# yanx27/PointASNL

Hardware: AMD Instinct MI355X
Metric: point-clouds/sec fwd (Bx1024 pts, ModelNet40 cls) (higher is better)
Workload: dtype f32; 1 GPU; configs[1]: ModelNet40 pointasnl_cls, 1024 pts, batch=64/GPU, seeded random weights; global_batch=64, parallelism=batch-shard x1, RCCL all-gather of logits, pipeline=prefetch, hip_graph=True, prefix_forked_at=start, prefix_levels=2, settle_replays=40, hip_hw_queues=4

## Files before the change

### pointasnl_amd/csrc/grouping.hip

```cpp
#include <math.h>
#include <stdlib.h>
#include <algorithm>
#include "common.hpp"

namespace pasnl {

constexpr int SEARCH_TILE = 2048;
constexpr int SEARCH_WAVES = 4;

__device__ __forceinline__ void stage_tile(const float* __restrict__ cloud, int n, int base, int cnt, float* sx, float* sy,
                                           float* sz) {
  const float* src = cloud + (size_t)base * 3;
  for (int f = threadIdx.x; f < cnt * 3; f += SEARCH_WAVES * 64) {
    float v = src[f];
    int p = f / 3, c = f - p * 3;
    (c == 0 ? sx : (c == 1 ? sy : sz))[p] = v;
  }
}

template <int QW>
__global__ __launch_bounds__(SEARCH_WAVES * 64) void ball_query_kernel(int n, int m, float thr2, int nsample,
                                                                      const float* __restrict__ xyz1,
                                                                      const float* __restrict__ xyz2,
                                                                      int* __restrict__ idx, int* __restrict__ pts_cnt) {
  extern __shared__ __attribute__((aligned(16))) char smem[];
  float* sx = reinterpret_cast<float*>(smem);
  float* sy = sx + SEARCH_TILE;
  float* sz = sy + SEARCH_TILE;
  int* hits = reinterpret_cast<int*>(sz + SEARCH_TILE);

  const int lane = threadIdx.x & 63, wave = threadIdx.x >> 6;
  const int bi = blockIdx.y;
  const float* cloud = xyz1 + (size_t)bi * n * 3;
  const int q0 = (blockIdx.x * SEARCH_WAVES + wave) * QW;

  float qx[QW], qy[QW], qz[QW];
  int cnt[QW], first[QW];
#pragma unroll
  for (int q = 0; q < QW; ++q) {
    int j = q0 + q;
    bool ok = j < m;
    const float* p = xyz2 + ((size_t)bi * m + (ok ? j : 0)) * 3;
    qx[q] = p[0]; qy[q] = p[1]; qz[q] = p[2];
    cnt[q] = ok ? 0 : nsample;
    first[q] = 0;
  }

  for (int base = 0; base < n; base += SEARCH_TILE) {
    int tcnt = min(SEARCH_TILE, n - base);
    __syncthreads();
    stage_tile(cloud, n, base, tcnt, sx, sy, sz);
    __syncthreads();
#pragma unroll
    for (int q = 0; q < QW; ++q) {
      int c = cnt[q];
      if (c >= nsample) continue;
      int* hq = hits + (size_t)(wave * QW + q) * nsample;
      for (int it = 0; it < tcnt; it += 64) {
        int p = it + lane;
        bool in = p < tcnt;
        float d2 = dist2(qx[q], qy[q], qz[q], in ? sx[p] : 0.f, in ? sy[p] : 0.f, in ? sz[p] : 0.f);
        bool hit = in && (d2 < thr2);
        unsigned long long mask = __ballot(hit);
        if (mask) {
          if (c == 0) first[q] = base + it + (int)__builtin_ctzll(mask);
          int rank = __builtin_amdgcn_mbcnt_hi((unsigned)(mask >> 32), __builtin_amdgcn_mbcnt_lo((unsigned)mask, 0u));
          int slot = c + rank;
          if (hit && slot < nsample) hq[slot] = base + it + lane;
          c += (int)__builtin_popcountll(mask);
          if (c >= nsample) { c = nsample; break; }
        }
      }
      cnt[q] = c;
    }
  }
#pragma unroll
  for (int q = 0; q < QW; ++q) {
    int j = q0 + q;
    if (j >= m) continue;
    const int* hq = hits + (size_t)(wave * QW + q) * nsample;
    int* o = idx + ((size_t)bi * m + j) * nsample;
    int c = cnt[q], pad = c > 0 ? first[q] : 0;
    for (int s = lane; s < nsample; s += 64) o[s] = s < c ? hq[s] : pad;
    if (lane == 0) pts_cnt[(size_t)bi * m + j] = c;
  }
}

int ball_grid_launch(int b, int n, int m, float radius, float thr2, int nsample, const float* xyz1, const float* xyz2, int* idx,
                     int* pts_cnt, hipStream_t stream);

template <int SLOTS>
struct KnnList {
  float d[SLOTS];
  int i[SLOTS];
};

template <int SLOTS>
__device__ __forceinline__ void knn_insert(KnnList<SLOTS>& L, float cd, int ck, int lane) {
  int pos = 0;
#pragma unroll
  for (int s = 0; s < SLOTS; ++s) pos += (int)__builtin_popcountll(__ballot(L.d[s] <= cd));
  float carry_d = 0.f;
  int carry_i = 0;
#pragma unroll
  for (int s = 0; s < SLOTS; ++s) {
    float top_d = readlane_f(L.d[s], 63);
    int top_i = __builtin_amdgcn_readlane(L.i[s], 63);
    float sd = wave_shr1_f(L.d[s]);
    int si = wave_shr1_i(L.i[s]);
    if (lane == 0) { sd = carry_d; si = carry_i; }
    int r = s * 64 + lane;
    if (r > pos) { L.d[s] = sd; L.i[s] = si; }
    if (r == pos) { L.d[s] = cd; L.i[s] = ck; }
    carry_d = top_d;
    carry_i = top_i;
  }
}

template <int SLOTS, int QW, typename IdxT>
__global__ __launch_bounds__(SEARCH_WAVES * 64) void knn_kernel(int n, int m, int k, const float* __restrict__ support,
                                                               const float* __restrict__ queries, IdxT* __restrict__ idx,
                                                               float* __restrict__ dist_out, const KnnTieFlags flags) {
  __shared__ float sx[SEARCH_TILE], sy[SEARCH_TILE], sz[SEARCH_TILE];
  const int lane = threadIdx.x & 63, wave = threadIdx.x >> 6;
  const int bi = blockIdx.y;
  const float* cloud = support + (size_t)bi * n * 3;
  const int q0 = (blockIdx.x * SEARCH_WAVES + wave) * QW;

  float qx[QW], qy[QW], qz[QW], tau[QW];
  float tie_tau[QW];
  const bool flagging = flags.nflag != nullptr;
  KnnList<SLOTS> L[QW];
  const int ks = (k - 1) >> 6, kl = (k - 1) & 63;
#pragma unroll
  for (int q = 0; q < QW; ++q) {
    int j = min(q0 + q, m - 1);
    const float* p = queries + ((size_t)bi * m + j) * 3;
    qx[q] = p[0]; qy[q] = p[1]; qz[q] = p[2];
    tau[q] = INFINITY;
    tie_tau[q] = -1.f;
#pragma unroll
    for (int s = 0; s < SLOTS; ++s) { L[q].d[s] = INFINITY; L[q].i[s] = 0; }
  }

  for (int base = 0; base < n; base += SEARCH_TILE) {
    int tcnt = min(SEARCH_TILE, n - base);
    __syncthreads();
    stage_tile(cloud, n, base, tcnt, sx, sy, sz);
    __syncthreads();
    for (int it = 0; it < tcnt; it += 64) {
      int p = it + lane;
      bool in = p < tcnt;
      float x = in ? sx[p] : 0.f, y = in ? sy[p] : 0.f, z = in ? sz[p] : 0.f;
      float dq[QW];
      dist2_multi<QW>(qx, qy, qz, x, y, z, dq);
#pragma unroll
      for (int q = 0; q < QW; ++q) {
        float d = dq[q];
        unsigned long long mask = __ballot(in && d < tau[q]);
        if (flagging && __ballot(in && d == tau[q]) != 0ull) tie_tau[q] = tau[q];
        while (mask) {
          int src = (int)__builtin_ctzll(mask);
          mask &= mask - 1;
          float cd = readlane_f(d, src);
          if (cd < tau[q]) {
            knn_insert<SLOTS>(L[q], cd, base + it + src, lane);
            float t = INFINITY;
#pragma unroll
            for (int s = 0; s < SLOTS; ++s)
              if (s == ks) t = readlane_f(L[q].d[s], kl);
            if (t == tau[q]) tie_tau[q] = t;
            tau[q] = t;
          } else if (cd == tau[q]) {
            tie_tau[q] = cd;
          }
        }
      }
    }
  }
#pragma unroll
  for (int q = 0; q < QW; ++q) {
    int j = q0 + q;
    if (j >= m) continue;
    size_t o = ((size_t)bi * m + j) * k;
    bool tie = flagging && tie_tau[q] == tau[q];
#pragma unroll
    for (int s = 0; s < SLOTS; ++s) {
      int r = s * 64 + lane;
      if (r < k) {
        idx[o + r] = (IdxT)L[q].i[s];
        if (dist_out) dist_out[o + r] = L[q].d[s];
      }
      if (flagging) {
        float prev = wave_shr1_f(L[q].d[s]);
        if (lane == 0) prev = s > 0 ? readlane_f(L[q].d[s > 0 ? s - 1 : 0], 63) : -1.f;
        tie = tie || __ballot(r >= 1 && r < k && L[q].d[s] == prev) != 0ull;
      }
    }
    if (tie) knn_flag_query(flags, bi, m, j, lane);
  }
}

constexpr int KNN2_CAP = 128;

template <int R, int QW, typename IdxT>
__global__ __launch_bounds__(SEARCH_WAVES * 64) void knn2_kernel(int n, int m, int k, const float* __restrict__ support,
                                                                const float* __restrict__ queries, IdxT* __restrict__ idx,
                                                                float* __restrict__ dist_out, const KnnTieFlags flags) {
  __shared__ float sx[SEARCH_TILE], sy[SEARCH_TILE], sz[SEARCH_TILE];
  __shared__ unsigned long long cand[SEARCH_WAVES * QW][KNN2_CAP];
  const int lane = threadIdx.x & 63, wave = threadIdx.x >> 6;
  const int bi = blockIdx.y;
  const float* cloud = support + (size_t)bi * n * 3;
  const int q0 = (blockIdx.x * SEARCH_WAVES + wave) * QW;
  constexpr uint32_t INF_BITS = 0x7f800000u;

  float qx[QW], qy[QW], qz[QW];
  uint32_t m1[QW], m2[QW];
#pragma unroll
  for (int q = 0; q < QW; ++q) {
    int j = min(q0 + q, m - 1);
    const float* p = queries + ((size_t)bi * m + j) * 3;
    qx[q] = p[0]; qy[q] = p[1]; qz[q] = p[2];
    m1[q] = INF_BITS; m2[q] = INF_BITS;
  }
  for (int base = 0; base < n; base += SEARCH_TILE) {
    int tcnt = min(SEARCH_TILE, n - base);
    __syncthreads();
    stage_tile(cloud, n, base, tcnt, sx, sy, sz);
    __syncthreads();
    for (int it = 0; it < tcnt; it += 64) {
      int p = it + lane;
      bool in = p < tcnt;
      const float x = sx[p], y = sy[p], z = sz[p];
      float dq[QW];
      dist2_multi<QW>(qx, qy, qz, x, y, z, dq);
#pragma unroll
      for (int q = 0; q < QW; ++q) {
        uint32_t di = in ? __float_as_uint(dq[q]) : INF_BITS;
        if (R == 2) m2[q] = min(m2[q], max(m1[q], di));
        m1[q] = min(m1[q], di);
      }
    }
  }
  uint32_t U[QW];
#pragma unroll
  for (int q = 0; q < QW; ++q) {
    uint32_t mv[R];
    mv[0] = m1[q];
    if (R == 2) mv[1] = m2[q];
    wave_bitonic_sort<R, uint32_t>(mv, lane);
    uint32_t u = 0;
#pragma unroll
    for (int r = 0; r < R; ++r)
      if (r == ((k - 1) >> 6)) u = (uint32_t)__builtin_amdgcn_readlane((int)mv[r], (k - 1) & 63);
    U[q] = u;
  }
  int cnt[QW];
#pragma unroll
  for (int q = 0; q < QW; ++q) cnt[q] = 0;
  for (int base = 0; base < n; base += SEARCH_TILE) {
    int tcnt = min(SEARCH_TILE, n - base);
    if (n > SEARCH_TILE) {
      __syncthreads();
      stage_tile(cloud, n, base, tcnt, sx, sy, sz);
      __syncthreads();
    }
    for (int it = 0; it < tcnt; it += 64) {
      int p = it + lane;
      bool in = p < tcnt;
      const float x = sx[p], y = sy[p], z = sz[p];
      float dq[QW];
      dist2_multi<QW>(qx, qy, qz, x, y, z, dq);
#pragma unroll
      for (int q = 0; q < QW; ++q) {
        uint32_t di = __float_as_uint(dq[q]);
        bool c = in && di <= U[q];
        unsigned long long mask = __ballot(c);
        if (mask) {
          int rank = __builtin_amdgcn_mbcnt_hi((unsigned)(mask >> 32), __builtin_amdgcn_mbcnt_lo((unsigned)mask, 0u));
          int slot = cnt[q] + rank;
          if (c && slot < KNN2_CAP) cand[wave * QW + q][slot] = ((unsigned long long)di << 32) | (uint32_t)(base + p);
          cnt[q] += (int)__builtin_popcountll(mask);
        }
      }
    }
  }
  bool overflow = false;
#pragma unroll
  for (int q = 0; q < QW; ++q) {
    const int j = q0 + q;
    const int c = cnt[q];
    if (c > KNN2_CAP) { overflow = overflow || (j < m); continue; }
    if (j >= m) continue;
    const unsigned long long* cb = cand[wave * QW + q];
    const size_t o = ((size_t)bi * m + j) * k;
    if (c <= 64) {
      unsigned long long key[1];
      key[0] = lane < c ? cb[lane] : ~0ull;
      wave_bitonic_sort<1, unsigned long long>(key, lane);
      if (lane < k) {
        idx[o + lane] = (IdxT)(uint32_t)key[0];
        if (dist_out) dist_out[o + lane] = __uint_as_float((uint32_t)(key[0] >> 32));
      }
      if (flags.nflag && knn_sorted_has_tie(key[0], ~0ull, k, lane)) knn_flag_query(flags, bi, m, j, lane);
    } else {
      unsigned long long key[2];
      key[0] = cb[lane];
      key[1] = 64 + lane < c ? cb[64 + lane] : ~0ull;
      wave_bitonic_sort<2, unsigned long long>(key, lane);
      if (lane < k) {
        idx[o + lane] = (IdxT)(uint32_t)key[0];
        if (dist_out) dist_out[o + lane] = __uint_as_float((uint32_t)(key[0] >> 32));
      }
      if (flags.nflag && knn_sorted_has_tie(key[0], key[1], k, lane)) knn_flag_query(flags, bi, m, j, lane);
    }
  }
  if (!__syncthreads_or(overflow ? 1 : 0)) return;
  float tau[QW], tie_tau[QW];
  KnnList<1> L[QW];
  bool todo[QW];
#pragma unroll
  for (int q = 0; q < QW; ++q) {
    todo[q] = cnt[q] > KNN2_CAP && (q0 + q) < m;
    tau[q] = INFINITY;
    tie_tau[q] = -1.f;
    L[q].d[0] = INFINITY;
    L[q].i[0] = 0;
  }
  for (int base = 0; base < n; base += SEARCH_TILE) {
    int tcnt = min(SEARCH_TILE, n - base);
    __syncthreads();
    stage_tile(cloud, n, base, tcnt, sx, sy, sz);
    __syncthreads();
    for (int it = 0; it < tcnt; it += 64) {
      int p = it + lane;
      bool in = p < tcnt;
      float x = in ? sx[p] : 0.f, y = in ? sy[p] : 0.f, z = in ? sz[p] : 0.f;
#pragma unroll
      for (int q = 0; q < QW; ++q) {
        if (!todo[q]) continue;
        float d = dist2(qx[q], qy[q], qz[q], x, y, z);
        unsigned long long mask = __ballot(in && d < tau[q]);
        if (__ballot(in && d == tau[q]) != 0ull) tie_tau[q] = tau[q];
        while (mask) {
          int src = (int)__builtin_ctzll(mask);
          mask &= mask - 1;
          float cd = readlane_f(d, src);
          if (cd < tau[q]) {
            knn_insert<1>(L[q], cd, base + it + src, lane);
            const float t = readlane_f(L[q].d[0], k - 1);
            if (t == tau[q]) tie_tau[q] = t;
            tau[q] = t;
          } else if (cd == tau[q]) {
            tie_tau[q] = cd;
          }
        }
      }
    }
  }
#pragma unroll
  for (int q = 0; q < QW; ++q) {
    if (!todo[q]) continue;
    size_t o = ((size_t)bi * m + q0 + q) * k;
    if (lane < k) {
      idx[o + lane] = (IdxT)L[q].i[0];
      if (dist_out) dist_out[o + lane] = L[q].d[0];
    }
    if (flags.nflag) {
      const float prev = wave_shr1_f(L[q].d[0]);
      if (tie_tau[q] == tau[q] || __ballot(lane >= 1 && lane < k && L[q].d[0] == prev) != 0ull) knn_flag_query(flags, bi, m, q0 + q, lane);
    }
  }
}

template <int VEC>
__global__ __launch_bounds__(256) void group_point_kernel(int n, int c, long rows_per_batch, long total_chunks,
                                                         const float* __restrict__ points, const int* __restrict__ idx,
                                                         float* __restrict__ out) {
  const int cpr = c / VEC;
  for (long g = (long)blockIdx.x * 256 + threadIdx.x; g < total_chunks; g += (long)gridDim.x * 256) {
    long row = g / cpr;
    int ch = (int)(g - row * cpr);
    long bi = row / rows_per_batch;
    int a = idx[row];
    const float* src = points + ((size_t)bi * n + a) * c + (size_t)ch * VEC;
    float* dst = out + (size_t)row * c + (size_t)ch * VEC;
    if constexpr (VEC == 4) {
      *reinterpret_cast<float4*>(dst) = *reinterpret_cast<const float4*>(src);
    } else {
      *dst = *src;
    }
  }
}

__global__ __launch_bounds__(256) void group_point_grad_kernel(int n, int c, long rows_per_batch, long total,
                                                              const float* __restrict__ grad_out,
                                                              const int* __restrict__ idx, float* __restrict__ grad_points) {
  for (long e = (long)blockIdx.x * 256 + threadIdx.x; e < total; e += (long)gridDim.x * 256) {
    long row = e / c;
    int l = (int)(e - row * c);
    long bi = row / rows_per_batch;
    int a = idx[row];
    atomicAdd(&grad_points[((size_t)bi * n + a) * c + l], grad_out[e]);
  }
}

template <int T>
__global__ __launch_bounds__(T) void sa_group_kernel(int n, int c, int m, int k, const float* __restrict__ xyz,
                                                    const float* __restrict__ feature, const int* __restrict__ idx,
                                                    const float* __restrict__ new_xyz, float* __restrict__ new_point,
                                                    float* __restrict__ skip_max) {
  extern __shared__ __attribute__((aligned(16))) char smem[];
  int* sidx = reinterpret_cast<int*>(smem);
  float* part = reinterpret_cast<float*>(sidx + k);
  const int W = 6 + c;
  const int R = T / W;
  const long g = blockIdx.x;
  const long bi = g / m;
  const int t = threadIdx.x;
  for (int s = t; s < k; s += T) sidx[s] = idx[g * k + s];
  __syncthreads();
  const float* cx = xyz + (size_t)bi * n * 3;
  const float* cf = feature + (size_t)bi * n * c;
  float* out = new_point + (size_t)g * k * W;
  if (W > T) {
    for (int col = t; col < W; col += T) {
      const float centre = col < 3 ? new_xyz[g * 3 + col] : 0.f;
      float mx = -INFINITY;
      for (int s = 0; s < k; ++s) {
        const int i = sidx[s];
        float v;
        if (col < 3) v = cx[(size_t)i * 3 + col] - centre;
        else if (col < 6) v = cx[(size_t)i * 3 + (col - 3)];
        else v = cf[(size_t)i * c + (col - 6)];
        out[(size_t)s * W + col] = v;
        mx = fmaxf(mx, v);
      }
      skip_max[g * W + col] = mx;
    }
    return;
  }
  const int col = t % W, r0 = t / W;
  const bool active = r0 < R;
  float centre = 0.f;
  if (active && col < 3) centre = new_xyz[g * 3 + col];
  float mx = -INFINITY;
  if (active) {
    for (int s = r0; s < k; s += R) {
      const int i = sidx[s];
      float v;
      if (col < 3) v = cx[(size_t)i * 3 + col] - centre;
      else if (col < 6) v = cx[(size_t)i * 3 + (col - 3)];
      else v = cf[(size_t)i * c + (col - 6)];
      out[(size_t)s * W + col] = v;
      mx = fmaxf(mx, v);
    }
    part[r0 * W + col] = mx;
  }
  __syncthreads();
  if (t < W) {
    float v = part[t];
    for (int r = 1; r < R; ++r) v = fmaxf(v, part[r * W + t]);
    skip_max[g * W + t] = v;
  }
}

constexpr int GL_THREADS = 1024;

__global__ __launch_bounds__(GL_THREADS) void grad_lists_kernel(int n, long entries, const int* __restrict__ idx,
                                                               int* __restrict__ start, int* __restrict__ list) {
  extern __shared__ __attribute__((aligned(16))) char smem[];
  int* cnt = reinterpret_cast<int*>(smem);
  __shared__ int wsum[GL_THREADS / 64];
  const int tid = threadIdx.x, lane = tid & 63, wave = tid >> 6;
  const long bi = blockIdx.x;
  const int* ix = idx + bi * entries;
  for (int t = tid; t < n; t += GL_THREADS) cnt[t] = 0;
  __syncthreads();
  for (long e = tid; e < entries; e += GL_THREADS) {
    const int t = ix[e];
    if (t >= 0 && t < n) atomicAdd(&cnt[t], 1);
  }
  __syncthreads();
  const int per = (n + GL_THREADS - 1) / GL_THREADS;
  int sum = 0;
  for (int j = 0; j < per; ++j) {
    const int t = tid * per + j;
    if (t < n) sum += cnt[t];
  }
  int incl = sum;
#pragma unroll
  for (int off = 1; off < 64; off <<= 1) {
    int o = __shfl_up(incl, off);
    if (lane >= off) incl += o;
  }
  if (lane == 63) wsum[wave] = incl;
  __syncthreads();
  int base = incl - sum;
  for (int w = 0; w < wave; ++w) base += wsum[w];
  int* st = start + bi * (n + 1);
  for (int j = 0; j < per; ++j) {
    const int t = tid * per + j;
    if (t < n) {
      const int c = cnt[t];
      cnt[t] = base;
      st[t] = base;
      base += c;
    }
  }
  if (tid == GL_THREADS - 1) st[n] = base;
  __syncthreads();
  int* ls = list + bi * entries;
  for (long e = tid; e < entries; e += GL_THREADS) {
    const int t = ix[e];
    if (t >= 0 && t < n) ls[atomicAdd(&cnt[t], 1)] = (int)e;
  }
}

__global__ __launch_bounds__(256) void grad_segsum_kernel(int n, int c, long entries, int rep, const float* __restrict__ src,
                                                         const float* __restrict__ weight, const int* __restrict__ start,
                                                         const int* __restrict__ list, float* __restrict__ dst, long rows) {
  const int lane = threadIdx.x & 63;
  const long r = (long)blockIdx.x * 4 + (threadIdx.x >> 6);
  if (r >= rows) return;
  const long bi = r / n;
  const int t = (int)(r - bi * n);
  const int lo = start[bi * (n + 1) + t], hi = start[bi * (n + 1) + t + 1];
  const int* ls = list + bi * entries;
  float* out = dst + r * c;
  constexpr int CH = 8;
  for (int c0 = 0; c0 < c; c0 += CH * 64) {
    float acc[CH];
#pragma unroll
    for (int q = 0; q < CH; ++q) acc[q] = 0.f;
    uint32_t prev = 0;
    bool first = true;
    for (int done = lo; done < hi;) {
      uint32_t key[2];
      key[0] = 0xffffffffu;
      for (int base = lo; base < hi; base += 64) {
        uint32_t cand = 0xffffffffu;
        if (base + lane < hi) {
          const uint32_t e = (uint32_t)ls[base + lane];
          if (first || e > prev) cand = e;
        }
        key[1] = cand;
        wave_bitonic_sort<2, uint32_t>(key, lane);
      }
      const int take = min(64, hi - done);
      for (int j = 0; j < take; ++j) {
        const uint32_t e = (uint32_t)__builtin_amdgcn_readlane((int)key[0], j);
        const long ge = bi * entries + e;
        const float* row = src + (ge / rep) * c + c0 + lane;
        const float w = weight ? weight[ge] : 1.f;
#pragma unroll
        for (int q = 0; q < CH; ++q) {
          if (c0 + q * 64 + lane < c) {
            const float v = row[q * 64];
            acc[q] = acc[q] + (weight ? v * w : v);
          }
        }
      }
      prev = (uint32_t)__builtin_amdgcn_readlane((int)key[0], take - 1);
      first = false;
      done += take;
    }
#pragma unroll
    for (int q = 0; q < CH; ++q)
      if (c0 + q * 64 + lane < c) out[c0 + q * 64 + lane] = acc[q];
  }
}

__global__ __launch_bounds__(256) void take_neighbor0_kernel(int n, int c, int m, int k, long total, const float* __restrict__ xyz,
                                                            const float* __restrict__ feature, const int* __restrict__ idx,
                                                            float* __restrict__ new_xyz, float* __restrict__ new_feature) {
  const int w = 3 + c;
  for (long e = (long)blockIdx.x * 256 + threadIdx.x; e < total; e += (long)gridDim.x * 256) {
    const long row = e / w;
    const int col = (int)(e - row * w);
    const long bi = row / m;
    const int i = idx[row * k];
    const float v = col < 3 ? xyz[((size_t)bi * n + i) * 3 + col] : feature[((size_t)bi * n + i) * c + (col - 3)];
    new_feature[e] = v;
    if (col < 3) new_xyz[row * 3 + col] = v;
  }
}

__global__ __launch_bounds__(256) void max_pool_rows_kernel(int n, int c, const float* __restrict__ x, float* __restrict__ out,
                                                            long out_stride) {
  __shared__ float part[4][64];
  const int lane = threadIdx.x & 63, wave = threadIdx.x >> 6;
  const int col = blockIdx.x * 64 + lane;
  const bool ok = col < c;
  const float* p = x + (size_t)blockIdx.y * n * c + (ok ? col : 0);
  float m0 = -INFINITY, m1 = -INFINITY, m2 = -INFINITY, m3 = -INFINITY;
  int s = wave;
  for (; s + 12 < n; s += 16) {
    float a = p[(size_t)s * c], b = p[(size_t)(s + 4) * c], d = p[(size_t)(s + 8) * c], e = p[(size_t)(s + 12) * c];
    m0 = fmaxf(m0, a); m1 = fmaxf(m1, b); m2 = fmaxf(m2, d); m3 = fmaxf(m3, e);
  }
  for (; s < n; s += 4) m0 = fmaxf(m0, p[(size_t)s * c]);
  part[wave][lane] = fmaxf(fmaxf(m0, m1), fmaxf(m2, m3));
  __syncthreads();
  if (wave == 0 && ok)
    out[(size_t)blockIdx.y * out_stride + col] = fmaxf(fmaxf(part[0][lane], part[1][lane]), fmaxf(part[2][lane], part[3][lane]));
}

__global__ __launch_bounds__(256) void select_top_k_kernel(int n, int k, long rows, const float* __restrict__ dist,
                                                          int* __restrict__ outi, float* __restrict__ out) {
  const int lane = threadIdx.x & 63;
  long row = (long)blockIdx.x * 4 + (threadIdx.x >> 6);
  if (row >= rows) return;
  const float* src = dist + (size_t)row * n;
  float* pd = out + (size_t)row * n;
  int* pi = outi + (size_t)row * n;
  for (int s = lane; s < n; s += 64) { pd[s] = src[s]; pi[s] = s; }
  asm volatile("s_waitcnt vmcnt(0)" ::: "memory");
  for (int s = 0; s < k && s < n; ++s) {
    float bv = INFINITY;
    int bp = 0x7fffffff;
    for (int t = s + lane; t < n; t += 64) {
      float v = __hip_atomic_load(&pd[t], __ATOMIC_RELAXED, __HIP_MEMORY_SCOPE_AGENT);
      if (v < bv) { bv = v; bp = t; }
    }
#pragma unroll
    for (int off = 32; off >= 1; off >>= 1) {
      float ov = __shfl_xor(bv, off);
      int op = __shfl_xor(bp, off);
      if (ov < bv || (ov == bv && op < bp)) { bv = ov; bp = op; }
    }
    int mn = (bp == 0x7fffffff) ? s : bp;
    if (mn != s && lane == 0) {
      float vs = __hip_atomic_load(&pd[s], __ATOMIC_RELAXED, __HIP_MEMORY_SCOPE_AGENT);
      int is = __hip_atomic_load(&pi[s], __ATOMIC_RELAXED, __HIP_MEMORY_SCOPE_AGENT);
      int im = __hip_atomic_load(&pi[mn], __ATOMIC_RELAXED, __HIP_MEMORY_SCOPE_AGENT);
      __hip_atomic_store(&pd[mn], vs, __ATOMIC_RELAXED, __HIP_MEMORY_SCOPE_AGENT);
      __hip_atomic_store(&pd[s], bv, __ATOMIC_RELAXED, __HIP_MEMORY_SCOPE_AGENT);
      __hip_atomic_store(&pi[mn], is, __ATOMIC_RELAXED, __HIP_MEMORY_SCOPE_AGENT);
      __hip_atomic_store(&pi[s], im, __ATOMIC_RELAXED, __HIP_MEMORY_SCOPE_AGENT);
    }
    asm volatile("s_waitcnt vmcnt(0)" ::: "memory");
  }
}

}

using namespace pasnl;

static int grid_for(long total) {
  long g = (total + 255) / 256;
  return (int)(g < 1 ? 1 : (g > 8192 ? 8192 : g));
}

static float ball_threshold(float r) {
  float t = r * r;
  if (!(t < INFINITY)) return INFINITY;
  while (sqrtf(t) >= r && t > 0.f) t = nextafterf(t, -INFINITY);
  while (sqrtf(t) < r) t = nextafterf(t, INFINITY);
  return t;
}

extern "C" int pasnl_query_ball_point(int b, int n, int m, float radius, int nsample, const float* xyz1, const float* xyz2,
                                      int* idx, int* pts_cnt, pasnl_stream_t stream) {
  PASNL_REQUIRE(radius > 0.f, PASNL_EINVAL);
  PASNL_REQUIRE(nsample > 0, PASNL_EINVAL);
  PASNL_REQUIRE(b >= 0 && n > 0 && m >= 0, PASNL_EINVAL);
  if (b == 0 || m == 0) return PASNL_OK;
  PASNL_REQUIRE(xyz1 && xyz2 && idx && pts_cnt, PASNL_ENULL);
  PASNL_REQUIRE(b <= 65535, PASNL_EUNSUPPORTED);
  constexpr int QW = 4;
  float thr2 = (radius > 1e-20f) ? ball_threshold(radius) : 0.f;
  const int rc = ball_grid_launch(b, n, m, radius, thr2, nsample, xyz1, xyz2, idx, pts_cnt, pasnl_hip_stream(stream));
  if (rc != PASNL_EUNSUPPORTED) return rc;
  size_t lds = (size_t)SEARCH_TILE * 12 + (size_t)SEARCH_WAVES * QW * nsample * sizeof(int);
  PASNL_REQUIRE(lds <= LDS_MAX_BYTES, PASNL_EUNSUPPORTED);
  int qpb = SEARCH_WAVES * QW;
  if (launch(ball_query_kernel<QW>, dim3((m + qpb - 1) / qpb, b), dim3(SEARCH_WAVES * 64), lds, pasnl_hip_stream(stream), n, m, thr2,
             nsample, xyz1, xyz2, idx, pts_cnt) != PASNL_OK)
    return PASNL_ELAUNCH;
  return pasnl_launch_status();
}

template <int SLOTS, int QW>
static int knn_launch(int b, int n, int m, int k, const float* support, const float* queries, void* idx, int idx_is_i64,
                      float* dist2, pasnl::KnnTieFlags flags, hipStream_t st) {
  int qpb = SEARCH_WAVES * QW;
  dim3 grid((m + qpb - 1) / qpb, b), block(SEARCH_WAVES * 64);
  with_index_type(idx_is_i64, [&](auto tag) {
    using T = decltype(tag);
    hipLaunchKernelGGL((knn_kernel<SLOTS, QW, T>), grid, block, 0, st, n, m, k, support, queries, static_cast<T*>(idx), dist2, flags);
  });
  return pasnl_launch_status();
}

extern "C" int pasnl_knn_batch(int b, int n, int m, int k, const float* support, const float* queries, void* idx,
                               int idx_is_i64, float* dist2, pasnl_stream_t stream) {
  return pasnl::knn_brute_launch(b, n, m, k, support, queries, idx, idx_is_i64, dist2, pasnl::KnnTieFlags{nullptr, nullptr},
                                 pasnl_hip_stream(stream));
}

int pasnl::knn_brute_launch(int b, int n, int m, int k, const float* support, const float* queries, void* idx, int idx_is_i64,
                            float* dist2, pasnl::KnnTieFlags flags, hipStream_t st) {
  PASNL_REQUIRE(b >= 0 && n > 0 && m >= 0 && k > 0, PASNL_EINVAL);
  PASNL_REQUIRE(k <= n, PASNL_EINVAL);
  PASNL_REQUIRE(k <= PASNL_KNN_MAX_K, PASNL_EUNSUPPORTED);
  if (b == 0 || m == 0) return PASNL_OK;
  PASNL_REQUIRE(support && queries && idx, PASNL_ENULL);
  PASNL_REQUIRE(b <= 65535, PASNL_EUNSUPPORTED);
  if (k <= 64 && !(k <= 16 && n > 2048)) {
    const long nq = (long)b * m;
    constexpr long min_waves = 8192;
    const int qw = nq >= 4L * min_waves ? 4 : (nq >= 2L * min_waves ? 2 : 1);
    dim3 grid((m + SEARCH_WAVES * qw - 1) / (SEARCH_WAVES * qw), b), block(SEARCH_WAVES * 64);
    with_index_type(idx_is_i64, [&](auto tag) {
      using T = decltype(tag);
      auto kern = k <= 32 ? (qw == 4 ? knn2_kernel<1, 4, T> : qw == 2 ? knn2_kernel<1, 2, T> : knn2_kernel<1, 1, T>)
                          : (qw == 4 ? knn2_kernel<2, 4, T> : qw == 2 ? knn2_kernel<2, 2, T> : knn2_kernel<2, 1, T>);
      hipLaunchKernelGGL(kern, grid, block, 0, st, n, m, k, support, queries, static_cast<T*>(idx), dist2, flags);
    });
    return pasnl_launch_status();
  }
  if (k <= 64) return knn_launch<1, 4>(b, n, m, k, support, queries, idx, idx_is_i64, dist2, flags, st);
  if (k <= 128) return knn_launch<2, 2>(b, n, m, k, support, queries, idx, idx_is_i64, dist2, flags, st);
  return knn_launch<4, 1>(b, n, m, k, support, queries, idx, idx_is_i64, dist2, flags, st);
}

extern "C" int pasnl_group_point(int b, int n, int c, int m, int nsample, const float* points, const int* idx, float* out,
                                 pasnl_stream_t stream) {
  PASNL_REQUIRE(b >= 0 && n > 0 && c > 0 && m >= 0 && nsample >= 0, PASNL_EINVAL);
  long rows_per_batch = (long)m * nsample;
  long rows = (long)b * rows_per_batch;
  if (rows == 0) return PASNL_OK;
  PASNL_REQUIRE(points && idx && out, PASNL_ENULL);
  hipStream_t st = pasnl_hip_stream(stream);
  bool vec4 = (c % 4 == 0) && ((reinterpret_cast<uintptr_t>(points) | reinterpret_cast<uintptr_t>(out)) % 16 == 0);
  if (vec4) {
    long chunks = rows * (c / 4);
    hipLaunchKernelGGL(group_point_kernel<4>, dim3(grid_for(chunks)), dim3(256), 0, st, n, c, rows_per_batch, chunks, points,
                       idx, out);
  } else {
    long chunks = rows * c;
    hipLaunchKernelGGL(group_point_kernel<1>, dim3(grid_for(chunks)), dim3(256), 0, st, n, c, rows_per_batch, chunks, points,
                       idx, out);
  }
  return pasnl_launch_status();
}

extern "C" int pasnl_sa_group(int b, int n, int c, int m, int k, const float* xyz, const float* feature, const int* idx,
                              const float* new_xyz, float* new_point, float* skip_max, pasnl_stream_t stream) {
  PASNL_REQUIRE(b >= 0 && n > 0 && c > 0 && m >= 0 && k > 0, PASNL_EINVAL);
  const int W = 6 + c;
  long groups = (long)b * m;
  if (groups == 0) return PASNL_OK;
  PASNL_REQUIRE(groups < (1L << 31), PASNL_EUNSUPPORTED);
  PASNL_REQUIRE(xyz && feature && idx && new_xyz && new_point && skip_max, PASNL_ENULL);
  hipStream_t st = pasnl_hip_stream(stream);
  if (W <= 256) {
    size_t lds = (size_t)k * 4 + (size_t)(256 / W) * W * 4;
    if (launch(sa_group_kernel<256>, dim3((unsigned)groups), dim3(256), lds, st, n, c, m, k, xyz, feature, idx, new_xyz, new_point,
               skip_max) != PASNL_OK)
      return PASNL_ELAUNCH;
  } else {
    size_t lds = (size_t)k * 4 + (size_t)(W <= 512 ? (512 / W) * W : 0) * 4;
    if (launch(sa_group_kernel<512>, dim3((unsigned)groups), dim3(512), lds, st, n, c, m, k, xyz, feature, idx, new_xyz, new_point,
               skip_max) != PASNL_OK)
      return PASNL_ELAUNCH;
  }
  return pasnl_launch_status();
}

extern "C" int pasnl_group_point_grad(int b, int n, int c, int m, int nsample, const float* grad_out, const int* idx,
                                      float* grad_points, pasnl_stream_t stream) {
  PASNL_REQUIRE(b >= 0 && n > 0 && c > 0 && m >= 0 && nsample >= 0, PASNL_EINVAL);
  if (b == 0) return PASNL_OK;
  PASNL_REQUIRE(grad_points, PASNL_ENULL);
  hipStream_t st = pasnl_hip_stream(stream);
  if (hipMemsetAsync(grad_points, 0, (size_t)b * n * c * sizeof(float), st) != hipSuccess) return PASNL_ELAUNCH;
  long rows_per_batch = (long)m * nsample;
  long total = (long)b * rows_per_batch * c;
  if (total == 0) return PASNL_OK;
  PASNL_REQUIRE(grad_out && idx, PASNL_ENULL);
  hipLaunchKernelGGL(group_point_grad_kernel, dim3(grid_for(total)), dim3(256), 0, st, n, c, rows_per_batch, total, grad_out,
                     idx, grad_points);
  return pasnl_launch_status();
}

static size_t grad_ws_bytes(int b, int n, long entries) {
  return ((size_t)b * (n + 1) + (size_t)b * entries) * sizeof(int);
}

extern "C" size_t pasnl_grad_workspace_bytes(int b, int n, long entries) {
  if (b <= 0 || n <= 0 || entries < 0) return 0;
  return grad_ws_bytes(b, n, entries);
}

static int grad_det(int b, int n, int c, long entries, int rep, const float* src, const float* weight, const int* idx,
                    float* dst, void* ws, size_t ws_bytes, hipStream_t st) {
  PASNL_REQUIRE(b >= 0 && n > 0 && c > 0 && entries >= 0, PASNL_EINVAL);
  if (b == 0) return PASNL_OK;
  PASNL_REQUIRE(dst, PASNL_ENULL);
  PASNL_REQUIRE(entries == 0 || (src && idx), PASNL_ENULL);
  PASNL_REQUIRE(ws && ws_bytes >= grad_ws_bytes(b, n, entries), PASNL_EWORKSPACE);
  PASNL_REQUIRE((size_t)n * sizeof(int) <= 150 * 1024 && entries < (1L << 31), PASNL_EUNSUPPORTED);
  int* start = static_cast<int*>(ws);
  int* list = start + (size_t)b * (n + 1);
  size_t lds = (size_t)n * sizeof(int);
  if (launch(grad_lists_kernel, dim3(b), dim3(GL_THREADS), lds, st, n, entries, idx, start, list) != PASNL_OK) return PASNL_ELAUNCH;
  long rows = (long)b * n;
  hipLaunchKernelGGL(grad_segsum_kernel, dim3((unsigned)((rows + 3) / 4)), dim3(256), 0, st, n, c, entries, rep, src, weight, start,
                     list, dst, rows);
  return pasnl_launch_status();
}

extern "C" int pasnl_gather_point_grad_det(int b, int n, int m, const float* out_g, const int* idx, float* inp_g, void* ws,
                                           size_t ws_bytes, pasnl_stream_t stream) {
  PASNL_REQUIRE(m >= 0, PASNL_EINVAL);
  return grad_det(b, n, 3, m, 1, out_g, nullptr, idx, inp_g, ws, ws_bytes, pasnl_hip_stream(stream));
}

extern "C" int pasnl_group_point_grad_det(int b, int n, int c, int m, int nsample, const float* grad_out, const int* idx,
                                          float* grad_points, void* ws, size_t ws_bytes, pasnl_stream_t stream) {
  PASNL_REQUIRE(m >= 0 && nsample >= 0, PASNL_EINVAL);
  return grad_det(b, n, c, (long)m * nsample, 1, grad_out, nullptr, idx, grad_points, ws, ws_bytes, pasnl_hip_stream(stream));
}

extern "C" int pasnl_three_interpolate_grad_det(int b, int n, int c, int m, const float* grad_out, const int* idx,
                                                const float* weight, float* grad_points, void* ws, size_t ws_bytes,
                                                pasnl_stream_t stream) {
  PASNL_REQUIRE(n >= 0, PASNL_EINVAL);
  PASNL_REQUIRE(n == 0 || weight, PASNL_ENULL);
  return grad_det(b, m, c, 3L * n, 3, grad_out, weight, idx, grad_points, ws, ws_bytes, pasnl_hip_stream(stream));
}

extern "C" int pasnl_take_neighbor0(int b, int n, int c, int m, int k, const float* xyz, const float* feature, const int* idx,
                                    float* new_xyz, float* new_feature, pasnl_stream_t stream) {
  PASNL_REQUIRE(b >= 0 && n > 0 && c > 0 && m >= 0 && k > 0, PASNL_EINVAL);
  long total = (long)b * m * (3 + c);
  if (total == 0) return PASNL_OK;
  PASNL_REQUIRE(xyz && feature && idx && new_xyz && new_feature, PASNL_ENULL);
  hipLaunchKernelGGL(take_neighbor0_kernel, dim3(grid_for(total)), dim3(256), 0, pasnl_hip_stream(stream), n, c, m, k, total, xyz,
                     feature, idx, new_xyz, new_feature);
  return pasnl_launch_status();
}

extern "C" int pasnl_max_pool_rows_strided(int b, int n, int c, const float* x, float* out, long out_stride,
                                           pasnl_stream_t stream) {
  PASNL_REQUIRE(b >= 0 && n > 0 && c > 0 && out_stride >= c, PASNL_EINVAL);
  if (b == 0) return PASNL_OK;
  PASNL_REQUIRE(x && out, PASNL_ENULL);
  PASNL_REQUIRE(b <= 65535, PASNL_EUNSUPPORTED);
  hipLaunchKernelGGL(max_pool_rows_kernel, dim3((c + 63) / 64, b), dim3(256), 0, pasnl_hip_stream(stream), n, c, x, out,
                     out_stride);
  return pasnl_launch_status();
}

extern "C" int pasnl_max_pool_rows(int b, int n, int c, const float* x, float* out, pasnl_stream_t stream) {
  return pasnl_max_pool_rows_strided(b, n, c, x, out, c, stream);
}

extern "C" int pasnl_select_top_k(int b, int n, int m, int k, const float* dist, int* outi, float* out,
                                  pasnl_stream_t stream) {
  PASNL_REQUIRE(k > 0, PASNL_EINVAL);
  PASNL_REQUIRE(b >= 0 && n > 0 && m >= 0, PASNL_EINVAL);
  long rows = (long)b * m;
  if (rows == 0) return PASNL_OK;
  PASNL_REQUIRE(dist && outi && out, PASNL_ENULL);
  hipLaunchKernelGGL(select_top_k_kernel, dim3((unsigned)((rows + 3) / 4)), dim3(256), 0, pasnl_hip_stream(stream), n, k, rows,
                     dist, outi, out);
  return pasnl_launch_status();
}
```

Measured before the change: 58590 point-clouds/s.

## Keep kNN distances in registers for small clouds and compact candidates branch-free

For support clouds of up to 1024 points, the brute-force kNN kernel now loads the whole cloud into LDS once. It keeps each lane's per-query squared distances in a register array during the threshold pass, so the candidate pass reuses them instead of recomputing distances and re-reading LDS. Candidate collection becomes a fully unrolled ballot/mbcnt compaction, with non-hits and overflow writes sent to a sink area just past the cloud in LDS. The cost is much higher register pressure (up to 16×QW distances per lane), which may reduce occupancy or spill, and more template instantiations.

Result: faster. 59270 point-clouds/s, median of 6 (+1.2%).

```diff
diff --git a/pointasnl_amd/csrc/grouping.hip b/pointasnl_amd/csrc/grouping.hip
--- a/pointasnl_amd/csrc/grouping.hip
+++ b/pointasnl_amd/csrc/grouping.hip
@@ -202,11 +202,36 @@
 }
 
 constexpr int KNN2_CAP = 128;
-
-template <int R, int QW, typename IdxT>
+constexpr int KNN2_BLOCK = 4;
+
+template <int R, int QW, bool TAIL>
+__device__ __forceinline__ void knn2_resident_block(int g, int n, int lane, const float* sx, const float* sy, const float* sz,
+                                                    const float (&qx)[QW], const float (&qy)[QW], const float (&qz)[QW],
+                                                    uint32_t (*dr)[QW], uint32_t (&m1)[QW], uint32_t (&m2)[QW]) {
+#pragma unroll
+  for (int e = 0; e < KNN2_BLOCK; ++e) {
+    const int it = g * KNN2_BLOCK + e;
+    const int p = it * 64 + lane;
+    const float x = sx[p], y = sy[p], z = sz[p];
+    float dq[QW];
+    dist2_multi<QW>(qx, qy, qz, x, y, z, dq);
+#pragma unroll
+    for (int q = 0; q < QW; ++q) {
+      uint32_t di = __float_as_uint(dq[q]);
+      if (TAIL) di = p < n ? di : 0xffffffffu;
+      dr[it][q] = di;
+      if (R == 2) m2[q] = min(m2[q], max(m1[q], di));
+      m1[q] = min(m1[q], di);
+    }
+  }
+}
+
+template <int R, int QW, typename IdxT, int NIT = 0>
 __global__ __launch_bounds__(SEARCH_WAVES * 64) void knn2_kernel(int n, int m, int k, const float* __restrict__ support,
                                                                 const float* __restrict__ queries, IdxT* __restrict__ idx,
                                                                 float* __restrict__ dist_out, const KnnTieFlags flags) {
+  static_assert(NIT % KNN2_BLOCK == 0 && NIT * 64 + 128 <= SEARCH_TILE,
+                "the resident form is one LDS tile, walked in whole blocks, with 128 words behind the cloud to spare (pass 2)");
   __shared__ float sx[SEARCH_TILE], sy[SEARCH_TILE], sz[SEARCH_TILE];
   __shared__ unsigned long long cand[SEARCH_WAVES * QW][KNN2_CAP];
   const int lane = threadIdx.x & 63, wave = threadIdx.x >> 6;
@@ -224,7 +249,25 @@
     qx[q] = p[0]; qy[q] = p[1]; qz[q] = p[2];
     m1[q] = INF_BITS; m2[q] = INF_BITS;
   }
-  for (int base = 0; base < n; base += SEARCH_TILE) {
+  uint32_t dr[NIT > 0 ? NIT : 1][QW];
+  if constexpr (NIT > 0) {
+    stage_tile(cloud, n, 0, n, sx, sy, sz);
+    __syncthreads();
+#pragma unroll
+    for (int g = 0; g < NIT / KNN2_BLOCK; ++g) {
+      if ((g + 1) * KNN2_BLOCK * 64 <= n) {
+        knn2_resident_block<R, QW, false>(g, n, lane, sx, sy, sz, qx, qy, qz, dr, m1, m2);
+      } else if (g * KNN2_BLOCK * 64 < n) {
+        knn2_resident_block<R, QW, true>(g, n, lane, sx, sy, sz, qx, qy, qz, dr, m1, m2);
+      } else {
+#pragma unroll
+        for (int e = 0; e < KNN2_BLOCK; ++e)
+#pragma unroll
+          for (int q = 0; q < QW; ++q) dr[g * KNN2_BLOCK + e][q] = 0xffffffffu;
+      }
+    }
+  }
+  for (int base = 0; NIT == 0 && base < n; base += SEARCH_TILE) {
     int tcnt = min(SEARCH_TILE, n - base);
     __syncthreads();
     stage_tile(cloud, n, base, tcnt, sx, sy, sz);
@@ -259,7 +302,34 @@
   int cnt[QW];
 #pragma unroll
   for (int q = 0; q < QW; ++q) cnt[q] = 0;
-  for (int base = 0; base < n; base += SEARCH_TILE) {
+  if constexpr (NIT > 0) {
+    const int wave_u = __builtin_amdgcn_readfirstlane(wave);
+#pragma unroll
+    for (int q = 0; q < QW; ++q) {
+      unsigned long long hit[NIT];
+      int c = 0;
+#pragma unroll
+      for (int it = 0; it < NIT; ++it) {
+        hit[it] = __ballot(dr[it][q] <= U[q]);
+        c += (int)__builtin_popcountll(hit[it]);
+      }
+      cnt[q] = c;
+      const bool fits = c <= KNN2_CAP;
+      uint32_t* const sink0 = reinterpret_cast<uint32_t*>(sx) + NIT * 64;
+      uint32_t* const sink = sink0 + 2 * lane;
+      uint32_t* run = fits ? reinterpret_cast<uint32_t*>(cand[wave_u * QW + q]) : sink0;
+      const int step = fits ? 2 : 0;
+#pragma unroll
+      for (int it = 0; it < NIT; ++it) {
+        const int rank = __builtin_amdgcn_mbcnt_hi((unsigned)(hit[it] >> 32), __builtin_amdgcn_mbcnt_lo((unsigned)hit[it], 0u));
+        uint32_t* const dst = dr[it][q] <= U[q] ? run + 2 * rank : sink;
+        dst[0] = (uint32_t)(it * 64 + lane);
+        dst[1] = dr[it][q];
+        run += step * (int)__builtin_popcountll(hit[it]);
+      }
+    }
+  }
+  for (int base = 0; NIT == 0 && base < n; base += SEARCH_TILE) {
     int tcnt = min(SEARCH_TILE, n - base);
     if (n > SEARCH_TILE) {
       __syncthreads();
@@ -715,8 +785,13 @@
     dim3 grid((m + SEARCH_WAVES * qw - 1) / (SEARCH_WAVES * qw), b), block(SEARCH_WAVES * 64);
     with_index_type(idx_is_i64, [&](auto tag) {
       using T = decltype(tag);
-      auto kern = k <= 32 ? (qw == 4 ? knn2_kernel<1, 4, T> : qw == 2 ? knn2_kernel<1, 2, T> : knn2_kernel<1, 1, T>)
-                          : (qw == 4 ? knn2_kernel<2, 4, T> : qw == 2 ? knn2_kernel<2, 2, T> : knn2_kernel<2, 1, T>);
+      auto pick = [&](auto nit) {
+        constexpr int NIT = decltype(nit)::value;
+        return k <= 32 ? (qw == 4 ? knn2_kernel<1, 4, T, NIT> : qw == 2 ? knn2_kernel<1, 2, T, NIT> : knn2_kernel<1, 1, T, NIT>)
+                       : (qw == 4 ? knn2_kernel<2, 4, T, NIT> : qw == 2 ? knn2_kernel<2, 2, T, NIT> : knn2_kernel<2, 1, T, NIT>);
+      };
+      auto kern = n <= 512 ? pick(std::integral_constant<int, 8>{})
+                           : n <= 1024 ? pick(std::integral_constant<int, 16>{}) : pick(std::integral_constant<int, 0>{});
       hipLaunchKernelGGL(kern, grid, block, 0, st, n, m, k, support, queries, static_cast<T*>(idx), dist2, flags);
     });
     return pasnl_launch_status();
```
